# cvjena/mvlm

Hardware: NVIDIA B200
Metric: scans/sec (higher is better)
Workload: dtype bf16

## Files before the change

mvlm_b200/csrc/conv_epilogue.cuh:

```cuda
#pragma once
#include "conv_umma.cuh"

#include <type_traits>

#ifndef MVLM_FLOW_RES_BUDGET
#define MVLM_FLOW_RES_BUDGET 32
#endif

namespace mvlm {
namespace epi {

constexpr int kThreads = 352;
constexpr int kEpiWarps = 8;
constexpr int kTileW = 8;
constexpr int kMaxTileH = 32;
constexpr int kMTile = 128;
constexpr int kStageFloats = 16 * 36;
constexpr int kMaxCout = 256;
constexpr int kTraceTiles = 64;

enum : int { F_PRE = 1, F_RES1 = 2, F_RES2 = 4, F_RAW = 8, F_POST = 16, F_F32 = 32 , F_ARGMAX = 64,
              F_MID = 128 , F_POOL = 256 ,
              F_UP = 512 ,
              F_M64 = 1024 ,
              F_POST2 = 2048 ,
              F_POOLX = 4096 ,
              F_STAT = 8192  };
constexpr int F_HEAD = F_F32 | F_ARGMAX;

inline int feature_mask(const ConvEpilogue& e) {
  return (e.out_pre ? F_PRE : 0) | (e.res1 ? F_RES1 : 0) | (e.res2 ? F_RES2 : 0) | (e.out_raw ? F_RAW : 0) |
         (e.out_post ? F_POST : 0) | (e.out_f32 ? F_F32 : 0) | (e.argmax_keys ? F_ARGMAX : 0) |
         (e.mid_scale ? F_MID : 0) | (e.pool2 ? F_POOL : 0) | (e.res_up ? F_UP : 0) |
         (e.aux_mode == 1 ? F_POST2 : 0) | (e.aux_mode == 2 ? F_POOLX : 0);
}

#ifdef __CUDACC__

__device__ __forceinline__ uint32_t order_f32(float f) {
  const uint32_t b = __float_as_uint(f);
  return b ^ (static_cast<uint32_t>(static_cast<int32_t>(b) >> 31) | 0x80000000u);
}

__device__ __forceinline__ uint4 pack8(const float (&f)[8]) {
  __nv_bfloat162 a = __floats2bfloat162_rn(f[0], f[1]);
  __nv_bfloat162 b = __floats2bfloat162_rn(f[2], f[3]);
  __nv_bfloat162 c = __floats2bfloat162_rn(f[4], f[5]);
  __nv_bfloat162 d = __floats2bfloat162_rn(f[6], f[7]);
  uint4 r;
  r.x = *reinterpret_cast<uint32_t*>(&a);
// ... 81 lines not shown

struct EpiTrace {
  long long* trace = nullptr;
  int trace_i = 0;
  long long t0 = 0;
  bool on = false;
};
#define MVLM_EPI_TRACE(slot)                                                                              \
  do {                                                                                                    \
    if (tr.on && tr.trace && tr.trace_i < kTraceTiles) tr.trace[tr.trace_i * 16 + (slot)] = clock64() - tr.t0; \
  } while (0)

template <bool kFlow>
__device__ __forceinline__ uint4 load_res(const uint8_t* p) {
  if constexpr (kFlow) return __ldcg(reinterpret_cast<const uint4*>(p));
  else return *reinterpret_cast<const uint4*>(p);
}

template <int F, bool kFlow>
__device__ __forceinline__ void epilogue_tile(const ConvShape& s, const ConvEpilogue& e, const int tile_h,
                                              const ChannelParams& ep, const TileCoord& tc, const ImageSlots& is,
                                              uint64_t* t_full, const uint32_t parity, const uint32_t tmem_acc,
                                              float* stage, const int ew, const int lane_grp, const int lane,
                                              ArgmaxState& am, const bool prof, long long& w0, EpiTrace& tr) {
  constexpr bool WS = (F & F_M64) != 0;
  constexpr int kM = kMTile;
  constexpr int kChGrp = 32;
  constexpr int kPitch = 36;
  constexpr int kCols = 16;
  constexpr int kUnitRows = kCols / 8;
  static_assert(kCols * kPitch <= kStageFloats, "transpose buffer");
  const int rep_log2 = !WS ? 0 : (s.cout_pad <= 32 ? 2 : 1);
  const int n_cgrp = 4 >> rep_log2;
  const int cgrp = lane_grp & (n_cgrp - 1);
  const int replica = lane_grp >> (2 - rep_log2);
  const int n_units = max(1, tile_h / kUnitRows);
  const int upr = max(1, n_units >> rep_log2);
  const int upw = max(1, upr >> 1);
  const int u_local = (ew >> 2) * upw;
  const int u_begin = replica * upr + u_local;
  const int oh = s.h * e.up_sy, ow = s.w * e.up_sx;
  const int pj = lane >> 2;
  const int cq = (lane & 3) * 8;
  constexpr bool kBf16Out = (F & (F_PRE | F_RAW | F_POST)) != 0;
  const uint32_t rs_pre = static_cast<uint32_t>(s.w * e.pre_cs) * 2u, rs_res1 = static_cast<uint32_t>(s.w * e.res1_cs) * 2u;
  const uint32_t rs_res2 = static_cast<uint32_t>(s.w * e.res2_cs) * 2u;
  const uint32_t rs_up = static_cast<uint32_t>((s.w >> 1) * e.up_cs) * 2u;
// ... 187 lines not shown
        }
        if (r + 1 < upw) tmem_load(r + 1);
        if (y < s.h) {
          if (kBf16Out) {
            __syncwarp();
            if (r < 2) MVLM_EPI_TRACE(9 + 4 * r);
            uint4 pool_cur[2];
#pragma unroll
            for (int ip = 0; ip < 2; ++ip) {
              const int row = kUnitRows * r + ip;
              const bool valid = row < n_rows_ok;
              float f[8] = {0.f, 0.f, 0.f, 0.f, 0.f, 0.f, 0.f, 0.f};
              if (valid) {
                lds8(stage + (pj + 8 * ip) * kPitch + cq, f);
                if (F & F_PRE)
                  *reinterpret_cast<uint4*>(b_pre + static_cast<size_t>(row * rs_pre)) = affine_relu_pack8(f, pre_s, pre_t);
                if (F & F_RES1) add8(r1[r % kPref][ip], f);
                if (F & F_RES2) add8(r2[r % kPref][ip], f);
                if (F & F_UP) add8(ru[r % kPref][0], f);
              }
              if (F & (F_POOL | F_POOLX)) pool_cur[ip] = pack8(f);
              if (!(F & F_POOL) && valid) {
                if (F & F_RAW) *reinterpret_cast<uint4*>(b_raw + static_cast<size_t>(row * rs_raw)) = (F & F_POOLX) ? pool_cur[ip] : pack8(f);
                if (F & F_POST)
                  *reinterpret_cast<uint4*>(b_post + static_cast<size_t>(row * rs_post)) = affine_relu_pack8(f, post_s, post_t);
                if (F & F_POST2) {
                  float ax_s[8], ax_t[8], g[8] = {0.f, 0.f, 0.f, 0.f, 0.f, 0.f, 0.f, 0.f};
                  add8(pack8(f), g);
                  lds8(ep.mid_s + c0_ok, ax_s);
                  lds8(ep.mid_t + c0_ok, ax_t);
                  *reinterpret_cast<uint4*>(b_aux1 + static_cast<size_t>(row * rs_aux1)) = affine_relu_pack8(g, ax_s, ax_t);
                }
              }
            }
            if (r < 2) MVLM_EPI_TRACE(10 + 4 * r);
            if (F & (F_POOL | F_POOLX)) {
              {
                uint4 m = max_bf16x8(pool_cur[0], pool_cur[1]);
                uint4 o;
                o.x = __shfl_xor_sync(0xffffffffu, m.x, 4);
                o.y = __shfl_xor_sync(0xffffffffu, m.y, 4);
                o.z = __shfl_xor_sync(0xffffffffu, m.z, 4);
                o.w = __shfl_xor_sync(0xffffffffu, m.w, 4);
                m = max_bf16x8(m, o);
                const int prow = r;
                if (2 * prow < n_rows_ok && (pj & 1) == 0) {
                  if (F & F_POOL) {
                    if (F & F_RAW) *reinterpret_cast<uint4*>(b_raw + static_cast<size_t>(prow * rs_raw)) = m;
// ... 42 lines not shown
```

mvlm_b200/csrc/conv_umma.cu:

```cuda
#include "conv_epilogue.cuh"

#include <stdlib.h>

#include <algorithm>
#include <type_traits>
#include <atomic>

namespace mvlm {

namespace {

using namespace epi;
constexpr int kMaxHSlots = 4;
constexpr int kMaxWSlots = 12;
constexpr int kPoolBytes = 198 * 1024;

struct __align__(8) Barriers {
  uint64_t h_full[kMaxHSlots];
  uint64_t h_empty[kMaxHSlots];
  uint64_t w_full[kMaxWSlots];
  uint64_t w_empty[kMaxWSlots];
  uint64_t t_full[2];
  uint64_t t_empty[2];
  uint32_t tmem_base;
};
static_assert(sizeof(Barriers) <= 512, "barrier block");

struct EpiParams {
  float bias[kMaxCout];
  float mid_s[kMaxCout];
  float mid_t[kMaxCout];
  float pre_s[kMaxCout];
  float pre_t[kMaxCout];
  float post_s[kMaxCout];
  float post_t[kMaxCout];
};

constexpr int kSmemBytes = kPoolBytes + kEpiWarps * kStageFloats * 4 + 512 + static_cast<int>(sizeof(EpiParams)) +
                           1024 ;
static_assert(kSmemBytes <= 227 * 1024, "shared memory budget");

__device__ __forceinline__ TileCoord decode_tile(const ConvParams& p, int t) {
  TileCoord c;
  c.mt = t % p.n_nt;
  int r = t / p.n_nt;
  c.tx = r % p.tiles_x;
  r /= p.tiles_x;
  c.ty = r % p.tiles_y;
  c.img = r / p.tiles_y;
  return c;
}

struct TileIter {
  TileCoord c, d;
  int n_nt, tiles_x, tiles_y;
  __device__ __forceinline__ TileIter(const ConvParams& p, int t_begin, int t_step)
      : c(decode_tile(p, t_begin)), d(decode_tile(p, t_step)), n_nt(p.n_nt), tiles_x(p.tiles_x), tiles_y(p.tiles_y) {}
  __device__ __forceinline__ void next() {
// ... 2 lines not shown
    c.mt -= carry ? n_nt : 0;
    c.tx += d.tx + carry;
    carry = c.tx >= tiles_x ? 1 : 0;
    c.tx -= carry ? tiles_x : 0;
    c.ty += d.ty + carry;
    carry = c.ty >= tiles_y ? 1 : 0;
    c.ty -= carry ? tiles_y : 0;
    c.img += d.img + carry;
  }
};

template <int F>
__global__ void __launch_bounds__(kThreads, 1) conv_umma_kernel(const __grid_constant__ ConvParams p) {
  constexpr bool ARGMAX = (F & F_ARGMAX) != 0;
  extern __shared__ uint8_t smem_raw[];
  const uint32_t raw_addr = ptx::smem_u32(smem_raw);
  uint8_t* smem = smem_raw + ((1024u - (raw_addr & 1023u)) & 1023u);
  uint8_t* h_slots = smem;
  uint8_t* w_slots = smem + p.n_hslots * p.h_slot_bytes;
  float* stage_all = reinterpret_cast<float*>(smem + kPoolBytes);
  Barriers* bar = reinterpret_cast<Barriers*>(reinterpret_cast<uint8_t*>(stage_all) + kEpiWarps * kStageFloats * 4);
  EpiParams* ep = reinterpret_cast<EpiParams*>(reinterpret_cast<uint8_t*>(bar) + 512);

  const int warp = threadIdx.x >> 5;
  const int lane = threadIdx.x & 31;

  const ConvShape& s = p.s;
  const ConvEpilogue& e = p.e;
  const int n_chunks = (s.cin + 63) >> 6;
  const int n_hslots = p.n_hslots, n_wslots = p.n_wslots;
  const int halo_px = kTileW + s.kw - 1;
  const int halo_rows = p.tile_h + s.kh - 1;
  constexpr bool M64 = (F & F_M64) != 0;
  constexpr bool STAT = (F & F_STAT) != 0;
  constexpr int kM = M64 ? 64 : kMTile;
  const int w_rows = s.cout_pad < kM ? s.cout_pad : kM;
  const int mma_m = M64 ? (s.cout_pad <= 32 ? 32 : 64) : kMTile;
  const uint32_t w_tap_bytes = M64 ? 64u * 128u : ((static_cast<uint32_t>(w_rows) * 128u + 1023u) & ~1023u);
  const uint32_t w_slot_bytes = w_tap_bytes * static_cast<uint32_t>(M64 ? s.kh : 1);
  const bool w_stat = p.w_stationary != 0;

  int t_begin, t_end, t_step;
  if (ARGMAX) {
    const int per = (p.total_tiles + gridDim.x - 1) / gridDim.x;
    t_begin = blockIdx.x * per;
    t_end = min(p.total_tiles, t_begin + per);
    t_step = 1;
  } else {
    t_begin = blockIdx.x; t_end = p.total_tiles; t_step = gridDim.x;
  }

  for (int i = threadIdx.x; i < s.cout_pad; i += kThreads) {
    ep->bias[i] = e.bias ? e.bias[i] : 0.f;
    ep->mid_s[i] = e.mid_scale ? e.mid_scale[i] : (e.aux_scale ? e.aux_scale[i] : 1.f);
    ep->mid_t[i] = e.mid_scale ? e.mid_shift[i] : (e.aux_shift ? e.aux_shift[i] : 0.f);
    ep->pre_s[i] = e.out_pre ? e.pre_scale[i] : 0.f;
    ep->pre_t[i] = e.out_pre ? e.pre_shift[i] : 0.f;
    ep->post_s[i] = e.out_post ? e.post_scale[i] : 0.f;
    ep->post_t[i] = e.out_post ? e.post_shift[i] : 0.f;
  }
  if (warp == 0 && lane == 0) {
    ptx::tma_prefetch_desc(&p.tm_a);
    ptx::tma_prefetch_desc(&p.tm_b);
    if (p.tail) { ptx::tma_prefetch_desc(&p.tm_a2); ptx::tma_prefetch_desc(&p.tm_b2); }
    if (F & F_RES1) ptx::tma_prefetch_desc(&p.tm_r1);
    if (F & F_RES2) ptx::tma_prefetch_desc(&p.tm_r2);
    if (F & F_UP) ptx::tma_prefetch_desc(&p.tm_up);
    for (int i = 0; i < n_hslots; ++i) {
      ptx::mbar_init(&bar->h_full[i], 1);
      ptx::mbar_init(&bar->h_empty[i], 1);
    }
    for (int i = 0; i < n_wslots; ++i) {
      ptx::mbar_init(&bar->w_full[i], 1);
      ptx::mbar_init(&bar->w_empty[i], 1);
    }
    for (int i = 0; i < 2; ++i) {
      ptx::mbar_init(&bar->t_full[i], 1);
      ptx::mbar_init(&bar->t_empty[i], kEpiWarps);
    }
    ptx::fence_mbar_init();
  }
  if (warp == 1) {
    ptx::tmem_alloc(&bar->tmem_base, 512);
    ptx::tmem_relinquish();
  }
  ptx::tc_fence_before();
  __syncthreads();
  ptx::tc_fence_after();
  asm volatile("griddepcontrol.wait;" ::: "memory");
  asm volatile("griddepcontrol.launch_dependents;" ::: "memory");
// ... 18 lines not shown
        const int x0 = tc.tx * kTileW + s.x_off0;
        const int y0 = tc.ty * p.tile_h + s.y_off0;
        for (int c = 0; c < n_chunks; ++c) {
          const bool is_tail = p.tail != 0 && c == n_chunks - 1;
          const uint32_t row_b = is_tail ? static_cast<uint32_t>(p.tail) * 2u : 128u;
          timed_wait(&bar->h_empty[sh], ph ^ 1, prof, w0);
          ptx::mbar_expect_tx(&bar->h_full[sh], static_cast<uint32_t>(halo_rows * halo_px) * row_b);
          ptx::tma_load_4d(is_tail ? &p.tm_a2 : &p.tm_a, &bar->h_full[sh], h_slots + sh * p.h_slot_bytes, c * 64, x0, y0, tc.img);
          if (c == 0) MVLM_TRACE(0);
          if (++sh == n_hslots) { sh = 0; ph ^= 1; }
        }
        if constexpr ((F & (F_RES1 | F_RES2 | F_UP)) != 0) {
          const int xa = tc.tx * kTileW, ya = tc.ty * p.tile_h, c_lo = tc.mt * kM;
          if (F & F_RES1) ptx::tma_prefetch_l2_4d(&p.tm_r1, c_lo, xa, ya, tc.img);
          if (F & F_RES2) ptx::tma_prefetch_l2_4d(&p.tm_r2, c_lo, xa, ya, tc.img);
          if (F & F_UP) ptx::tma_prefetch_l2_4d(&p.tm_up, c_lo, xa >> 1, ya >> 1, tc.img);
        }
        ++trace_i;
      }
      if (prof) { p.prof[blockIdx.x * 8 + 0] = w0; p.prof[blockIdx.x * 8 + 7] = clock64() - t_kernel0; }
    }
  } else if (warp == 10) {
    if (ptx::elect_one() && (p.debug_mode & 1) == 0) {
      int sw = 0;
      uint32_t pw = 0;
      for (int t = t_begin; t < t_end; t += t_step) {
        const int mt = t % p.n_nt;
        for (int c = 0; c < n_chunks; ++c) {
          const bool is_tail = p.tail != 0 && c == n_chunks - 1;
          const void* tmb = is_tail ? &p.tm_b2 : &p.tm_b;
          const uint32_t row_b = is_tail ? static_cast<uint32_t>(p.tail) * 2u : 128u;
          const uint32_t wb = static_cast<uint32_t>(w_rows) * row_b;
          if constexpr (M64) {
            for (int kx = 0; kx < s.kw; ++kx) {
              if (!w_stat) timed_wait(&bar->w_empty[sw], pw ^ 1, prof, w1);
              ptx::mbar_expect_tx(&bar->w_full[sw], wb * static_cast<uint32_t>(s.kh));
              for (int ky = 0; ky < s.kh; ++ky)
                ptx::tma_load_2d(tmb, &bar->w_full[sw], w_slots + sw * w_slot_bytes + ky * w_tap_bytes,
                                 (kx * s.kh + ky) * s.cin + c * 64, mt * kM);
              if (++sw == n_wslots) { sw = 0; pw ^= 1; }
            }
          } else
          for (int tap = 0; tap < s.kw * s.kh; ++tap) {
            if (!w_stat) timed_wait(&bar->w_empty[sw], pw ^ 1, prof, w1);
            ptx::mbar_expect_tx(&bar->w_full[sw], wb);
            ptx::tma_load_2d(tmb, &bar->w_full[sw], w_slots + sw * w_slot_bytes, tap * s.cin + c * 64, mt * kM);
// ... 6 lines not shown
      }
      if (prof) p.prof[blockIdx.x * 8 + 1] = w1;
    }
  } else if (warp == 1) {
    if (ptx::elect_one()) {
      const uint32_t idesc = ptx::umma_idesc_bf16(mma_m, p.tile_h * kTileW);
      const bool live = (p.debug_mode & 1) == 0;
      const int n_kx = s.kw, n_ky = s.kh;
      const uint32_t tail_row_b = p.tail ? static_cast<uint32_t>(p.tail) * 2u : 128u;
      const uint32_t tail_swz = !p.tail ? 2u : (p.tail == 16 ? 6u : 4u);
      const uint64_t a_hi_full = static_cast<uint64_t>(((8u * 128u) >> 4) | (1u << 14) | (2u << 29)) << 32;
      const uint64_t b_hi_full = static_cast<uint64_t>(((static_cast<uint32_t>(halo_px) * 128u) >> 4) | (1u << 14) | (2u << 29)) << 32;
      const uint64_t a_hi_tail = static_cast<uint64_t>(((8u * tail_row_b) >> 4) | (1u << 14) | (tail_swz << 29)) << 32;
      const uint64_t b_hi_tail = static_cast<uint64_t>(((static_cast<uint32_t>(halo_px) * tail_row_b) >> 4) | (1u << 14) | (tail_swz << 29)) << 32;
      const uint32_t h_lo0 = (ptx::smem_u32(h_slots) >> 4) | (1u << 16), h_step = static_cast<uint32_t>(p.h_slot_bytes) >> 4;
      const uint32_t w_lo0 = (ptx::smem_u32(w_slots) >> 4) | (1u << 16), w_step = w_slot_bytes >> 4;
      const int last_chunk = n_chunks - 1;
      const int nk_last = (s.cin - last_chunk * 64) >= 64 ? 4 : ((s.cin - last_chunk * 64) >> 4);
      int sh = 0, sw = 0;
      uint32_t ph = 0, pw = 0;
      int acc = 0;
      uint32_t pacc = 0;
      bool w_wait = live;
      for (int t = t_begin; t < t_end; t += t_step) {
        timed_wait(&bar->t_empty[acc], pacc ^ 1, prof, w1);
        ptx::tc_fence_after();
        MVLM_TRACE(2);
        const uint32_t d = tmem_base + static_cast<uint32_t>(acc * 256);
        uint32_t accumulate = 0;
        for (int c = 0; c < n_chunks; ++c) {
          const bool is_tail = p.tail != 0 && c == last_chunk;
          const int nk = c == last_chunk ? nk_last : 4;
          const uint32_t rb16 = (is_tail ? tail_row_b : 128u) >> 4;
          const uint64_t a_hi = is_tail ? a_hi_tail : a_hi_full;
          const uint64_t b_hi = is_tail ? b_hi_tail : b_hi_full;
          const uint32_t ky_step = static_cast<uint32_t>(halo_px) * rb16;
          if (live) timed_wait(&bar->h_full[sh], ph, prof, w0);
          if (c == 0) MVLM_TRACE(3);
          uint32_t x_col = h_lo0 + static_cast<uint32_t>(sh) * h_step;
          if (STAT && !w_wait && (nk == 4 || nk == 2 || nk == 1)) {
            auto taps = [&](auto nk_c, auto kk_c) __attribute__((always_inline)) {
              constexpr int NK = decltype(nk_c)::value;
              constexpr int KK = decltype(kk_c)::value;
              constexpr uint32_t kRb16 = NK * 2;
              const uint32_t tap16 = M64 ? (64u * 128u >> 4) : w_step;
              const uint32_t w_base = w_lo0 + static_cast<uint32_t>(c * KK * KK) * tap16;
#pragma unroll
              for (int tap = 0; tap < KK * KK; ++tap) {
                const uint32_t x_lo = x_col + static_cast<uint32_t>(((tap % KK) * (kTileW + KK - 1) + tap / KK)) * kRb16;
                const uint32_t w_lo = w_base + static_cast<uint32_t>(tap) * tap16;
#pragma unroll
// ... 39 lines not shown
            uint32_t x_lo = x_col;
            for (int ky = 0; ky < n_ky; ++ky, x_lo += ky_step) {
              if (w_wait) timed_wait(&bar->w_full[sw], w_stat ? 0u : pw, prof, w0);
              const uint32_t w_lo = w_lo0 + static_cast<uint32_t>(sw) * w_step;
              auto mma = [&](int k, uint32_t en) __attribute__((always_inline)) {
                if constexpr (M64) ptx::umma_ws_bf16(d, a_hi | (w_lo + 2 * k), b_hi | (x_lo + 2 * k), idesc, en);
                else ptx::umma_bf16(d, a_hi | (w_lo + 2 * k), b_hi | (x_lo + 2 * k), idesc, en);
              };
              mma(0, accumulate);
              if (nk == 4) {
                mma(1, 1u); mma(2, 1u); mma(3, 1u);
              } else {
                for (int k = 1; k < nk; ++k) mma(k, 1u);
              }
              accumulate = 1;
              if (live && !w_stat) ptx::umma_commit(&bar->w_empty[sw]);
              if (++sw == n_wslots) { sw = 0; pw ^= 1; }
            }
          }
          if (live) ptx::umma_commit(&bar->h_empty[sh]);
          if (++sh == n_hslots) { sh = 0; ph ^= 1; }
        }
        ptx::umma_commit(&bar->t_full[acc]);
        MVLM_TRACE(4);
        ++trace_i;
        if (w_stat) w_wait = false;
        if (++acc == 2) { acc = 0; pacc ^= 1; }
      }
      if (prof) { p.prof[blockIdx.x * 8 + 2] = w0; p.prof[blockIdx.x * 8 + 3] = w1; p.prof[blockIdx.x * 8 + 4] = clock64() - t_kernel0; }
    }
  } else {
    float* stage = stage_all + (warp - 2) * kStageFloats;
    const ChannelParams cp = {ep->bias, ep->mid_s, ep->mid_t, ep->pre_s, ep->pre_t, ep->post_s, ep->post_t};
    int acc = 0;
    uint32_t pacc = 0;
    ArgmaxState am;
    EpiTrace tr;
    tr.trace = trace; tr.t0 = t_kernel0; tr.on = warp == 2 && lane == 0;
    TileIter it(p, t_begin, t_step);
    for (int t = t_begin; t < t_end; t += t_step, it.next()) {
      const TileCoord tc = it.c;
      const ImageSlots is = {tc.img, tc.img, tc.img, tc.img, tc.img, tc.img, tc.img, tc.img};
      tr.trace_i = trace_i;
      if (p.debug_mode & 2) {
        timed_wait(&bar->t_full[acc], pacc, prof, w0);
        ptx::tc_fence_after();
      } else {
        epilogue_tile<F, false>(s, e, p.tile_h, cp, tc, is, &bar->t_full[acc], pacc,
                                tmem_base + static_cast<uint32_t>(acc * 256), stage, warp - 2, warp & 3, lane, am, prof, w0,
                                tr);
      }
      ptx::tc_fence_before();
      __syncwarp();
      if (lane == 0) ptx::mbar_arrive(&bar->t_empty[acc]);
      if (warp == 2 && lane == 0) MVLM_TRACE(6);
      ++trace_i;
      if (++acc == 2) { acc = 0; pacc ^= 1; }
    }
    epilogue_argmax_flush<F>(s, e, warp & 3, lane, am);
    if (prof && warp == 2 && lane == 0) { p.prof[blockIdx.x * 8 + 5] = w0; p.prof[blockIdx.x * 8 + 6] = clock64() - t_kernel0; }
  }

#undef MVLM_TRACE
  ptx::tc_fence_before();
  __syncthreads();
  if (warp == 1) {
    ptx::tc_fence_after();
    ptx::tmem_dealloc(tmem_base, 512);
  }
}

typedef CUresult (*EncodeTiledFn)(CUtensorMap*, CUtensorMapDataType, cuuint32_t, void*,
                                  const cuuint64_t*, const cuuint64_t*, const cuuint32_t*,
                                  const cuuint32_t*, CUtensorMapInterleave, CUtensorMapSwizzle,
                                  CUtensorMapL2promotion, CUtensorMapFloatOOBfill);

EncodeTiledFn get_encode_fn() {
// ... 164 lines not shown
      cuuint32_t estr[4] = {1, 1, 1, 1};
      return enc(tm, CU_TENSOR_MAP_DATA_TYPE_BFLOAT16, 4, const_cast<__nv_bfloat16*>(base + co), gdim, gstr, box, estr,
                 CU_TENSOR_MAP_INTERLEAVE_NONE, CU_TENSOR_MAP_SWIZZLE_NONE, CU_TENSOR_MAP_L2_PROMOTION_L2_128B,
                 CU_TENSOR_MAP_FLOAT_OOB_FILL_NONE) == CUDA_SUCCESS;
    };
    const bool ok = res_map(&p.tm_r1, e.res1, e.res1_co, e.res1_cs, s.h, s.w, kTileW, tile_h) &&
                    res_map(&p.tm_r2, e.res2, e.res2_co, e.res2_cs, s.h, s.w, kTileW, tile_h) &&
                    res_map(&p.tm_up, e.res_up, e.up_co, e.up_cs, s.h >> 1, s.w >> 1, kTileW / 2, std::max(1, tile_h / 2));
    if (!ok) {
      set_error("conv_plan: cuTensorMapEncodeTiled(residual) failed (cout_pad=%d w=%d h=%d)", s.cout_pad, s.w, s.h);
      return MVLM_E_CUDA;
    }
  }
  p.tiles_x = ceil_div(s.w, kTileW);
  p.tiles_y = ceil_div(s.h, tile_h);
  p.n_nt = s.cout_pad <= 64 ? 1 : ceil_div(s.cout_pad, kMTile);
  p.total_tiles = s.n * p.tiles_x * p.tiles_y * p.n_nt;
  p.prof = nullptr;
  p.debug_mode = 0;
  *out = p;
  return MVLM_OK;
}

void conv_set_profile_buffer(long long* dev_buf) { g_prof_buf = dev_buf; }
void conv_set_debug_mode(int mode) { g_debug_mode = mode; }

int conv_launch(const ConvParams& p_in, cudaStream_t stream) {
  ConvParams p = p_in;
  p.prof = g_prof_buf;
  p.debug_mode = g_debug_mode;
  const ConvEpilogue& e = p.e;
  const int f = feature_mask(e);
  const bool m64 = p.s.cout_pad <= 64;
  const bool stat = m64 && p.w_stationary && p.s.kw == 3 && p.s.kh == 3;
#define MVLM_CASE_BOTH(FLAGS) \
  case (FLAGS):               \
    return m64 ? (stat ? launch_t<(FLAGS) | F_M64 | F_STAT>(p, stream) : launch_t<(FLAGS) | F_M64>(p, stream)) : launch_t<(FLAGS)>(p, stream)
#define MVLM_CASE_128(FLAGS) \
  case (FLAGS):              \
    if (!m64) return launch_t<(FLAGS)>(p, stream); \
    break
  if (f == F_ARGMAX && !m64 && p.w_stationary && p.s.kw == 2 && p.s.kh == 2) return launch_t<F_ARGMAX | F_STAT>(p, stream);
  switch (f) {
    MVLM_CASE_BOTH(F_PRE | F_RES1 | F_RAW | F_POST);
    MVLM_CASE_BOTH(F_PRE | F_RES1 | F_RAW);
    MVLM_CASE_BOTH(F_RES1 | F_RAW | F_POST);
    MVLM_CASE_BOTH(F_RES1 | F_RAW);
    MVLM_CASE_BOTH(F_RAW);
    MVLM_CASE_128(F_PRE);
    MVLM_CASE_128(F_RES1 | F_RES2 | F_RAW | F_POST);
    MVLM_CASE_128(F_ARGMAX);
    MVLM_CASE_BOTH(F_F32);
    MVLM_CASE_BOTH(F_F32 | F_ARGMAX);
    MVLM_CASE_BOTH(F_MID | F_PRE | F_POST);
    MVLM_CASE_BOTH(F_POOL | F_PRE | F_RES1 | F_RAW | F_POST);
    MVLM_CASE_BOTH(F_POOL | F_RES1 | F_RAW | F_POST);
    MVLM_CASE_BOTH(F_POOL | F_RAW);
    MVLM_CASE_128(F_PRE | F_RES1 | F_RES2 | F_RAW | F_POST);
    MVLM_CASE_BOTH(F_UP | F_PRE | F_RES1 | F_RAW | F_POST);
    MVLM_CASE_BOTH(F_UP | F_PRE | F_RES1 | F_RAW);
    MVLM_CASE_BOTH(F_UP | F_RES1 | F_RAW | F_POST);
    MVLM_CASE_BOTH(F_UP | F_RES1 | F_RAW);
    MVLM_CASE_BOTH(F_POST2 | F_PRE | F_RES1 | F_RAW | F_POST);
    MVLM_CASE_BOTH(F_POST2 | F_RES1 | F_RAW | F_POST);
// ... 12 lines not shown
```

mvlm_b200/csrc/conv_umma.cuh:

```cuda
#pragma once
#include "common.cuh"

namespace mvlm {

struct ConvEpilogue {
  const float* bias = nullptr;
  const float* mid_scale = nullptr;
  const float* mid_shift = nullptr;
  const float* pre_scale = nullptr;
  const float* pre_shift = nullptr;
  __nv_bfloat16* out_pre = nullptr;
  int pre_cs = 0, pre_co = 0;
  const __nv_bfloat16* res1 = nullptr;
  int res1_cs = 0, res1_co = 0;
  const __nv_bfloat16* res2 = nullptr;
  int res2_cs = 0, res2_co = 0;
  const __nv_bfloat16* res_up = nullptr;
  int up_cs = 0, up_co = 0;
  __nv_bfloat16* out_raw = nullptr;
  int raw_cs = 0, raw_co = 0;
  const float* post_scale = nullptr;
  const float* post_shift = nullptr;
  __nv_bfloat16* out_post = nullptr;
  int post_cs = 0, post_co = 0;
// ... 18 lines not shown
  int in_cs = 0;
  const __nv_bfloat16* wpacked = nullptr;
  int cout_pad = 0;
  int n_tile = 0;
  int kh = 3, kw = 3;
  int y_off0 = -1, x_off0 = -1;
};

struct alignas(64) ConvParams {
  CUtensorMap tm_a;
  CUtensorMap tm_b;
  CUtensorMap tm_a2;
  CUtensorMap tm_b2;
  CUtensorMap tm_r1, tm_r2, tm_up;
  int tail;
  ConvShape s;
  ConvEpilogue e;
  int tiles_x, tiles_y, n_nt, total_tiles;
  int tile_h;
  int h_slot_bytes, n_hslots, n_wslots;
  int w_stationary;
  long long* prof;
  int debug_mode;
};

int conv_plan(const ConvShape& s, const ConvEpilogue& e, ConvParams* out);
int conv_launch(const ConvParams& p, cudaStream_t stream);
constexpr int kConvTraceTiles = 64;
constexpr int kConvProfInts = 148 * 8 + kConvTraceTiles * 16;
void conv_set_profile_buffer(long long* dev_buf);
void conv_set_debug_mode(int mode);

}
```

mvlm_b200/csrc/hourglass.cu:

```cuda
#include "hourglass.cuh"

#include <math.h>
#include <stdlib.h>

#include <algorithm>

namespace mvlm {

namespace {

__global__ void fold_bn_kernel(const float* w, const float* b, const float* m, const float* v, float eps, int n,
                               float* scale, float* shift) {
  const int i = blockIdx.x * blockDim.x + threadIdx.x;
  if (i >= n) return;
  const float s = w[i] / sqrtf(v[i] + eps);
  scale[i] = s;
  shift[i] = b[i] - m[i] * s;
}

__global__ void pack_weight_kernel(const float* __restrict__ w, int cout, int cin, int k, int cout_pad, int cin_pad,
                                   __nv_bfloat16* __restrict__ out) {
  const long long total = 1ll * cout_pad * k * k * cin_pad;
  for (long long i = blockIdx.x * 1ll * blockDim.x + threadIdx.x; i < total; i += 1ll * gridDim.x * blockDim.x) {
    const int ci = static_cast<int>(i % cin_pad);
// ... 149 lines not shown
        ++j;
      }
    }
    size_t best = free_list.size();
    for (size_t j = 0; j < free_list.size(); ++j)
      if (free_list[j].bytes >= b.bytes && (best == free_list.size() || free_list[j].bytes < free_list[best].bytes)) best = j;
    if (best < free_list.size()) {
      b.offset = free_list[best].off;
      free_list[best].off += b.bytes;
      free_list[best].bytes -= b.bytes;
      if (free_list[best].bytes == 0) free_list.erase(free_list.begin() + best);
    } else {
      b.offset = top;
      top += b.bytes;
    }
    ws_needed_ = std::max(ws_needed_, b.offset + b.bytes);
    ws_needed_ = std::max(ws_needed_, top);
    live.push_back(id);
  }
}

static int op_out_rows(const NetOp& op) {
  switch (op.kind) {
    case NetOp::CONV: return op.is_head ? -1 : op.h;
    case NetOp::POOL: return op.h / 2;
    case NetOp::BNRELU: return op.h;
    default: return -1;
  }
}

void HourglassNet::push_op(const NetOp& op) {
  const int rows = op_out_rows(op);
  const bool in_window = flow_on_ && rows >= flow_lo_ && rows <= flow_hi_;
  if (!in_window) {
    cur_seg_ = -1;
  } else if (cur_seg_ < 0 || cur_seg_layers_ >= kFlowMaxLayers) {
    cur_seg_ = n_segs_++;
    cur_seg_layers_ = 0;
  }
  if (in_window) ++cur_seg_layers_;
  ops_.push_back(op);
  op_seg_.push_back(cur_seg_);
}

HourglassNet::T HourglassNet::alloc(int h, int w, int c) {
  T t;
  t.h = h; t.w = w; t.c = c;
// ... 95 lines not shown
    packed(wname + ".weight", cout, cin_real, k, cout_pad, cin, &dw);
    if (with_bias) bias(wname + ".bias", cout, cout_pad, &db);
  }
  if (!dry_) {
    ConvShape s;
    s.in = in.p; s.n = V_; s.h = in.h; s.w = in.w; s.cin = cin; s.in_cs = in.c;
    const __nv_bfloat16* wp;
    int rc = packed(wname + ".weight", cout, cin_real, k, cout_pad, cin, &wp);
    if (rc) return rc;
    s.wpacked = wp; s.cout_pad = cout_pad; s.n_tile = n_tile; s.kh = k; s.kw = k;
    s.y_off0 = -(k / 2); s.x_off0 = -(k / 2);
    if (with_bias) {
      rc = bias(wname + ".bias", cout, cout_pad, &e.bias);
      if (rc) return rc;
    }
    rc = conv_plan(s, e, &op.conv);
    if (rc) return rc;
  }
  push_op(op);
  return MVLM_OK;
}

int HourglassNet::rb(const std::string& p, T x, T a_in, T ar, int cin, int cout, const char* post_bn, T* post_act,
                     T* y_out, T* pool_raw, const T* up_low, const RbAux* aux) {
  const int h = a_in.h, w = a_in.w;
  T y = alloc(h, w, cout);
  T skip = x;
  int rc;
  if (cin != cout) {
    ConvEpilogue e;
    e.out_raw = y.p; e.raw_cs = cout; e.raw_co = 0;
    rc = emit_conv("rb.resample", ar, cin, p + ".resample.2", cout, cout, cout < 128 ? cout : 128, 1, e, false);
    if (rc) return rc;
    skip = y;
  }
  const float *ps = nullptr, *pt = nullptr;
  if (post_bn) {
    rc = bn(post_bn, cout, &ps, &pt);
    if (rc) return rc;
    *post_act = pool_raw ? alloc(h / 2, w / 2, cout) : alloc(h, w, cout);
  }
  if (pool_raw) *pool_raw = alloc(h / 2, w / 2, cout);
  const float *as = nullptr, *at = nullptr;
  if (aux) {
    rc = bn(aux->bn, cout, &as, &at);
    if (rc) return rc;
    *aux->out1 = aux->mode == 2 ? alloc(h / 2, w / 2, cout) : alloc(h, w, cout);
    if (aux->mode == 2) *aux->out2 = alloc(h / 2, w / 2, cout);
  }
  const int c1 = cout / 2, c2 = cout / 4;
  T a1 = alloc(h, w, c1);
  T a2 = alloc(h, w, c2);
// ... 158 lines not shown
  cudaStreamDestroy(build_stream_);
  build_stream_ = nullptr;
  if (rc) return rc;
  MVLM_CHECK_CUDA(ce);
  return MVLM_OK;
}

void HourglassNet::probe(const char* name, const T& t) {
  probes[name] = {t.p, t.h, t.w, t.c};
  if (layout_pass_ && keep_probes_ && t.p) {
    const size_t off = static_cast<size_t>(reinterpret_cast<const uint8_t*>(t.p) - kFakeBase);
    for (Buf& b : bufs_)
      if (b.fake_off == off) b.pinned = true;
  }
}

int HourglassNet::emit() {
  const int h = H_, w = W_, cin = cin_;
  ops_.clear(); flops_ = 0.0; probes.clear();
  op_seg_.clear(); segs_.clear(); seg_info_.clear(); cur_seg_ = -1; n_segs_ = 0; cur_seg_layers_ = 0;
  int rc;
  const int F = 256, h2 = h / 2, w2 = w / 2;

  T a_c2 = alloc(h, w, 64), ar_c2 = alloc(h, w, 64);
  T img16 = alloc(h, w, 16);
  {
    note_use(img16.p);
    NetOp op;
    op.kind = NetOp::STEM;
    op.out_raw = img16.p; op.h = h; op.w = w; op.c = cin;
    push_op(op);
    flops_ += 2.0 * 64 * cin * 9 * h * w;
    note_use(img16.p); note_use(a_c2.p); note_use(ar_c2.p);
    NetOp cv;
    cv.kind = NetOp::CONV;
    cv.tag = "conv1";
    cv.h = h; cv.w = w;
    if (layout_pass_) {
      param_alloc(sizeof(__nv_bfloat16) * 64 * 9 * 16);
      const float* dummy;
      bias("conv1.bias", 64, 64, &dummy);
      bn("bn1", 64, &dummy, &dummy);
      bn("conv2.bn1", 64, &dummy, &dummy);
      bn("conv2.resample.0", 64, &dummy, &dummy);
    }
    if (!dry_) {
      const float* w1 = nullptr;
      if ((rc = sd_get("conv1.weight", 64ll * cin * 9, &w1))) return rc;
      __nv_bfloat16* wp = static_cast<__nv_bfloat16*>(param_alloc(sizeof(__nv_bfloat16) * 64 * 9 * 16));
      MVLM_REQUIRE(wp, "hourglass: parameter arena exhausted (conv1)");
      pack_stem_weight_kernel<<<36, 256, 0, build_stream_>>>(w1, 64, cin, 64, wp);
      MVLM_CHECK_CUDA(cudaGetLastError());
      ConvShape s;
      s.in = img16.p; s.n = V_; s.h = h; s.w = w; s.cin = 16; s.in_cs = 16;
      s.wpacked = wp; s.cout_pad = 64; s.n_tile = 64; s.kh = 3; s.kw = 3; s.y_off0 = -1; s.x_off0 = -1;
      ConvEpilogue e;
      if ((rc = bias("conv1.bias", 64, 64, &e.bias))) return rc;
      if ((rc = bn("bn1", 64, &e.mid_scale, &e.mid_shift))) return rc;
      if ((rc = bn("conv2.bn1", 64, &e.pre_scale, &e.pre_shift))) return rc;
      if ((rc = bn("conv2.resample.0", 64, &e.post_scale, &e.post_shift))) return rc;
      e.out_pre = a_c2.p; e.pre_cs = 64; e.pre_co = 0;
      e.out_post = ar_c2.p; e.post_cs = 64; e.post_co = 0;
      if ((rc = conv_plan(s, e, &cv.conv))) return rc;
    }
    push_op(cv);
  }
  T none, y2, y3, r3, a3, a4, a_h1, ar4;
  T x1;
  if ((rc = rb("conv2", none, a_c2, ar_c2, 64, 128, "conv3.bn1", &a3, &y2, &x1))) return rc;
  probe("x1", x1);
  if (fuse_elt_) {
    RbAux aux = {1, "conv4.resample.0", &ar4, nullptr};
    if ((rc = rb("conv3", x1, a3, none, 128, 128, "conv4.bn1", &a4, &y3, nullptr, nullptr, &aux))) return rc;
    probe("y3", y3);
  } else {
    if ((rc = rb("conv3", x1, a3, none, 128, 128, "conv4.bn1", &a4, &y3))) return rc;
    probe("y3", y3);
    ar4 = alloc(h2, w2, 128);
    note_use(y3.p); note_use(ar4.p);
    NetOp op;
    op.kind = NetOp::BNRELU;
    op.in0 = y3.p; op.out_act = ar4.p; op.h = h2; op.w = w2; op.c = 128;
    if ((rc = bn("conv4.resample.0", 128, &op.scale, &op.shift))) return rc;
    push_op(op);
  }
  T p1, pa1, p2, pa2;
  RbAux aux4 = {2, "hg1.rb2.bn1", &p1, &pa1};
  if ((rc = rb("conv4", y3, a4, ar4, 128, F, "hg1.rb1.bn1", &a_h1, &r3, nullptr, nullptr, fuse_elt_ ? &aux4 : nullptr))) return rc;
  probe("r3", r3);
  T hg1;
  if ((rc = hourglass("hg1", r3, a_h1, &hg1, fuse_elt_ ? &p1 : nullptr, fuse_elt_ ? &pa1 : nullptr))) return rc;
  probe("hg1", hg1);
// ... 384 lines not shown
```

mvlm_b200/csrc/hourglass.cuh:

```cuda
#pragma once
#include <map>
#include <set>
#include <string>
#include <vector>

#include "conv_flow.cuh"
#include "conv_umma.cuh"
#include "stages.cuh"

namespace mvlm {

struct SdEntry {
  const float* p = nullptr;
  long long numel = -1;
};
typedef std::map<std::string, SdEntry> StateDict;

struct NetOp {
  enum Kind { CONV, POOL, BNRELU, STEM, MEMSET, PEAKS } kind;
  ConvParams conv;
  const __nv_bfloat16* in0 = nullptr;
  const __nv_bfloat16* in1 = nullptr;
  __nv_bfloat16* out_raw = nullptr;
  __nv_bfloat16* out_act = nullptr;
  const float* scale = nullptr;
  const float* shift = nullptr;
  int h = 0, w = 0, c = 0;
  void* ptr = nullptr;
  size_t bytes = 0;
  bool is_head = false;
  const char* tag = "";
};

class HourglassNet {
 public:
  HourglassNet() = default;
  ~HourglassNet();
  int build(const StateDict* sd, int n_landmarks, int cin, int n_views, int h, int w,
            void* workspace, size_t workspace_bytes, bool dry);
  int forward(const unsigned char* img_u8, const float* img_f32, float* out_heatmaps, float* out_peaks,
              cudaStream_t stream);
  int run_op(NetOp& op, const unsigned char* img_u8, const float* img_f32, float* out_heatmaps, float* out_peaks,
             cudaStream_t stream);
  int run_step(size_t i, const unsigned char* img_u8, const float* img_f32, float* out_heatmaps, float* out_peaks,
               cudaStream_t stream);
  int forward_graph(const unsigned char* img_u8, const float* img_f32, float* out_heatmaps, float* out_peaks,
                    cudaStream_t stream);

  int set_selection_method(int method);
  int forward_keys(const unsigned char* img_u8, const float* img_f32, unsigned long long* out_keys, cudaStream_t stream);

  int profile_ops(const unsigned char* img_u8, const float* img_f32, float* out_peaks, int reps, float* ms_out,
                  double* roles_out, int trace_op, long long* trace_out, cudaStream_t stream);
// ... 21 lines not shown
    bool pinned = false;
  };
  int emit();
  void note_use(const void* p);
  void note_conv(const void* in, const ConvEpilogue& e);
  void assign_offsets();
  void probe(const char* name, const T& t);
  void* param_alloc(size_t bytes);
  unsigned char* params_ = nullptr;
  size_t param_off_ = 0, param_cap_ = 0;
  std::set<std::string> bn_seen_;
  cudaStream_t build_stream_ = nullptr;
  static constexpr size_t kMaxGraphs = 8;
  std::vector<Buf> bufs_;
  size_t fake_off_ = 0, ws_needed_ = 0, next_buf_ = 0;
  bool layout_pass_ = false, keep_probes_ = false, reuse_ = true, fuse_elt_ = false;
  int bn(const std::string& name, int c, const float** scale, const float** shift);
  int packed(const std::string& name, int cout, int cin, int k, int cout_pad, int cin_pad, const __nv_bfloat16** out);
  int bias(const std::string& name, int cout, int cout_pad, const float** out);
  int emit_conv(const char* tag, T in, int cin, const std::string& wname, int cout, int cout_pad, int n_tile, int k,
                ConvEpilogue e, bool with_bias);
  struct RbAux { int mode; const char* bn; T* out1; T* out2; };
  int rb(const std::string& p, T x, T a_in, T ar, int cin, int cout, const char* post_bn, T* post_act, T* y_out,
         T* pool_raw = nullptr, const T* up_low = nullptr, const RbAux* aux = nullptr);
  int hourglass(const std::string& p, T x, T a_x, T* out, const T* in_pooled = nullptr, const T* in_pooled_act = nullptr);
  int emit_pool(T in, T out_raw, const char* bn_name, T out_act);

  void push_op(const NetOp& op);
  int build_segments();
  bool flow_on_ = false;
  int flow_lo_ = 1, flow_hi_ = 32;
  int cur_seg_layers_ = 0;
  int flow_tiles_ = 64;
  int flow_interleave_ = 3;
  int cur_seg_ = -1, n_segs_ = 0;
  std::vector<int> op_seg_;
  std::vector<FlowSegment> segs_;
  struct SegInfo { int batch = 1, n_layers = 0, first_op = -1; };
  std::vector<SegInfo> seg_info_;
  float* zeros_ = nullptr;
  float* ones_ = nullptr;

  const StateDict* sd_ = nullptr;
  int sd_get(const std::string& name, long long numel, const float** out) const;
  bool dry_ = true;
  int V_ = 0, H_ = 0, W_ = 0, L_ = 0, Lp_ = 0, cin_ = 0;
  uint8_t* ws_ = nullptr;
// ... 17 lines not shown
```

Before: 64.23.

## Chain conv1 with the conv2 1x1 resample GEMM inside one UMMA kernel

Fuses the stem's 3x3 conv1 with the following 1x1 resample conv. The post-activated tile is staged in swizzled shared memory, a second UMMA against preloaded W2 writes into a separate TMEM region, and a second epilogue pass stores the 128-channel result. This drops the separate resample launch and the global round trip of the activated intermediate. In exchange it adds more barriers, halves the accumulator column stride, and leaves less shared memory for the operand rings.

```diff
diff --git a/mvlm_b200/csrc/conv_epilogue.cuh b/mvlm_b200/csrc/conv_epilogue.cuh
--- a/mvlm_b200/csrc/conv_epilogue.cuh
+++ b/mvlm_b200/csrc/conv_epilogue.cuh
@@ -25,7 +25,8 @@
               F_M64 = 1024 ,
               F_POST2 = 2048 ,
               F_POOLX = 4096 ,
-              F_STAT = 8192  };
+              F_STAT = 8192 ,
+              F_CHAIN = 16384  };
 constexpr int F_HEAD = F_F32 | F_ARGMAX;
 
 inline int feature_mask(const ConvEpilogue& e) {
@@ -153,7 +154,8 @@
                                               const ChannelParams& ep, const TileCoord& tc, const ImageSlots& is,
                                               uint64_t* t_full, const uint32_t parity, const uint32_t tmem_acc,
                                               float* stage, const int ew, const int lane_grp, const int lane,
-                                              ArgmaxState& am, const bool prof, long long& w0, EpiTrace& tr) {
+                                              ArgmaxState& am, const bool prof, long long& w0, EpiTrace& tr,
+                                              uint8_t* stg = nullptr) {
   constexpr bool WS = (F & F_M64) != 0;
   constexpr int kM = kMTile;
   constexpr int kChGrp = 32;
@@ -387,8 +389,12 @@
               if (F & (F_POOL | F_POOLX)) pool_cur[ip] = pack8(f);
               if (!(F & F_POOL) && valid) {
                 if (F & F_RAW) *reinterpret_cast<uint4*>(b_raw + static_cast<size_t>(row * rs_raw)) = (F & F_POOLX) ? pool_cur[ip] : pack8(f);
-                if (F & F_POST)
+                if constexpr ((F & F_CHAIN) != 0) {
+                  const int n = (kUnitRows * u_begin + row) * kTileW + pj;
+                  *reinterpret_cast<uint4*>(stg + n * 128 + (((c0 >> 3) ^ pj) << 4)) = affine_relu_pack8(f, post_s, post_t);
+                } else if (F & F_POST) {
                   *reinterpret_cast<uint4*>(b_post + static_cast<size_t>(row * rs_post)) = affine_relu_pack8(f, post_s, post_t);
+                }
                 if (F & F_POST2) {
                   float ax_s[8], ax_t[8], g[8] = {0.f, 0.f, 0.f, 0.f, 0.f, 0.f, 0.f, 0.f};
                   add8(pack8(f), g);
diff --git a/mvlm_b200/csrc/conv_umma.cu b/mvlm_b200/csrc/conv_umma.cu
--- a/mvlm_b200/csrc/conv_umma.cu
+++ b/mvlm_b200/csrc/conv_umma.cu
@@ -14,6 +14,9 @@
 constexpr int kMaxHSlots = 4;
 constexpr int kMaxWSlots = 12;
 constexpr int kPoolBytes = 198 * 1024;
+constexpr int kChainWBytes = kMTile * 128;
+constexpr int kChainStageBytes = kMaxTileH * kTileW * 128;
+constexpr int kChainBytes = kChainWBytes + 2 * kChainStageBytes;
 
 struct __align__(8) Barriers {
   uint64_t h_full[kMaxHSlots];
@@ -22,6 +25,9 @@
   uint64_t w_empty[kMaxWSlots];
   uint64_t t_full[2];
   uint64_t t_empty[2];
+  uint64_t s_full[2], s_empty[2];
+  uint64_t r_full, r_empty;
+  uint64_t w2_full;
   uint32_t tmem_base;
 };
 static_assert(sizeof(Barriers) <= 512, "barrier block");
@@ -34,6 +40,7 @@
   float pre_t[kMaxCout];
   float post_s[kMaxCout];
   float post_t[kMaxCout];
+  float zero[kMTile];
 };
 
 constexpr int kSmemBytes = kPoolBytes + kEpiWarps * kStageFloats * 4 + 512 + static_cast<int>(sizeof(EpiParams)) +
@@ -82,6 +89,11 @@
   Barriers* bar = reinterpret_cast<Barriers*>(reinterpret_cast<uint8_t*>(stage_all) + kEpiWarps * kStageFloats * 4);
   EpiParams* ep = reinterpret_cast<EpiParams*>(reinterpret_cast<uint8_t*>(bar) + 512);
 
+  constexpr bool CHAIN = (F & F_CHAIN) != 0;
+  uint8_t* const c_w2 = smem + kPoolBytes - kChainBytes;
+  uint8_t* const c_stg = c_w2 + kChainWBytes;
+  constexpr uint32_t kAccCols = CHAIN ? 128u : 256u;
+
   const int warp = threadIdx.x >> 5;
   const int lane = threadIdx.x & 31;
 
@@ -116,9 +128,11 @@
     ep->mid_t[i] = e.mid_scale ? e.mid_shift[i] : (e.aux_shift ? e.aux_shift[i] : 0.f);
     ep->pre_s[i] = e.out_pre ? e.pre_scale[i] : 0.f;
     ep->pre_t[i] = e.out_pre ? e.pre_shift[i] : 0.f;
-    ep->post_s[i] = e.out_post ? e.post_scale[i] : 0.f;
-    ep->post_t[i] = e.out_post ? e.post_shift[i] : 0.f;
-  }
+    ep->post_s[i] = (e.out_post || CHAIN) ? e.post_scale[i] : 0.f;
+    ep->post_t[i] = (e.out_post || CHAIN) ? e.post_shift[i] : 0.f;
+  }
+  if (CHAIN)
+    for (int i = threadIdx.x; i < kMTile; i += kThreads) ep->zero[i] = 0.f;
   if (warp == 0 && lane == 0) {
     ptx::tma_prefetch_desc(&p.tm_a);
     ptx::tma_prefetch_desc(&p.tm_b);
@@ -126,6 +140,16 @@
     if (F & F_RES1) ptx::tma_prefetch_desc(&p.tm_r1);
     if (F & F_RES2) ptx::tma_prefetch_desc(&p.tm_r2);
     if (F & F_UP) ptx::tma_prefetch_desc(&p.tm_up);
+    if (CHAIN) {
+      ptx::tma_prefetch_desc(&p.tm_w2);
+      for (int i = 0; i < 2; ++i) {
+        ptx::mbar_init(&bar->s_full[i], kEpiWarps);
+        ptx::mbar_init(&bar->s_empty[i], 1);
+      }
+      ptx::mbar_init(&bar->r_full, 1);
+      ptx::mbar_init(&bar->r_empty, kEpiWarps);
+      ptx::mbar_init(&bar->w2_full, 1);
+    }
     for (int i = 0; i < n_hslots; ++i) {
       ptx::mbar_init(&bar->h_full[i], 1);
       ptx::mbar_init(&bar->h_empty[i], 1);
@@ -190,6 +214,10 @@
     }
   } else if (warp == 10) {
     if (ptx::elect_one() && (p.debug_mode & 1) == 0) {
+      if (CHAIN) {
+        ptx::mbar_expect_tx(&bar->w2_full, kChainWBytes);
+        ptx::tma_load_2d(&p.tm_w2, &bar->w2_full, c_w2, 0, 0);
+      }
       int sw = 0;
       uint32_t pw = 0;
       for (int t = t_begin; t < t_end; t += t_step) {
@@ -242,11 +270,28 @@
       int acc = 0;
       uint32_t pacc = 0;
       bool w_wait = live;
-      for (int t = t_begin; t < t_end; t += t_step) {
+      const uint32_t idesc2 = ptx::umma_idesc_bf16(kMTile, p.tile_h * kTileW);
+      const uint32_t w2_lo = (ptx::smem_u32(c_w2) >> 4) | (1u << 16);
+      const uint32_t stg_lo0 = (ptx::smem_u32(c_stg) >> 4) | (1u << 16);
+      auto chain_gemm = [&](int j) __attribute__((always_inline)) {
+        const int sb = j & 1;
+        timed_wait(&bar->s_full[sb], static_cast<uint32_t>(j >> 1) & 1u, prof, w0);
+        timed_wait(&bar->r_empty, static_cast<uint32_t>(j & 1) ^ 1u, prof, w1);
+        if (j == 0 && live) timed_wait(&bar->w2_full, 0u, prof, w0);
+        ptx::tc_fence_after();
+        const uint32_t b_lo = stg_lo0 + static_cast<uint32_t>(sb) * (kChainStageBytes >> 4);
+#pragma unroll
+        for (int k = 0; k < 4; ++k)
+          ptx::umma_bf16(tmem_base + 256u, a_hi_full | (w2_lo + 2 * k), a_hi_full | (b_lo + 2 * k), idesc2, k > 0 ? 1u : 0u);
+        ptx::umma_commit(&bar->s_empty[sb]);
+        ptx::umma_commit(&bar->r_full);
+      };
+      int j_tile = 0;
+      for (int t = t_begin; t < t_end; t += t_step, ++j_tile) {
         timed_wait(&bar->t_empty[acc], pacc ^ 1, prof, w1);
         ptx::tc_fence_after();
         MVLM_TRACE(2);
-        const uint32_t d = tmem_base + static_cast<uint32_t>(acc * 256);
+        const uint32_t d = tmem_base + static_cast<uint32_t>(acc) * kAccCols;
         uint32_t accumulate = 0;
         for (int c = 0; c < n_chunks; ++c) {
           const bool is_tail = p.tail != 0 && c == last_chunk;
@@ -332,11 +377,13 @@
           if (++sh == n_hslots) { sh = 0; ph ^= 1; }
         }
         ptx::umma_commit(&bar->t_full[acc]);
+        if (CHAIN && j_tile > 0) chain_gemm(j_tile - 1);
         MVLM_TRACE(4);
         ++trace_i;
         if (w_stat) w_wait = false;
         if (++acc == 2) { acc = 0; pacc ^= 1; }
       }
+      if (CHAIN && j_tile > 0) chain_gemm(j_tile - 1);
       if (prof) { p.prof[blockIdx.x * 8 + 2] = w0; p.prof[blockIdx.x * 8 + 3] = w1; p.prof[blockIdx.x * 8 + 4] = clock64() - t_kernel0; }
     }
   } else {
@@ -347,22 +394,42 @@
     ArgmaxState am;
     EpiTrace tr;
     tr.trace = trace; tr.t0 = t_kernel0; tr.on = warp == 2 && lane == 0;
+    ConvShape s2 = s;
+    s2.cout_pad = kMTile;
+    ConvEpilogue e2;
+    e2.out_raw = p.out2; e2.raw_cs = kMTile;
+    const ChannelParams cp2 = {ep->zero, ep->zero, ep->zero, ep->zero, ep->zero, ep->zero, ep->zero};
+    EpiTrace tr2;
     TileIter it(p, t_begin, t_step);
-    for (int t = t_begin; t < t_end; t += t_step, it.next()) {
+    int j_tile = 0;
+    for (int t = t_begin; t < t_end; t += t_step, it.next(), ++j_tile) {
       const TileCoord tc = it.c;
       const ImageSlots is = {tc.img, tc.img, tc.img, tc.img, tc.img, tc.img, tc.img, tc.img};
+      const int sb = j_tile & 1;
       tr.trace_i = trace_i;
+      if (CHAIN) timed_wait(&bar->s_empty[sb], (static_cast<uint32_t>(j_tile >> 1) & 1u) ^ 1u, prof, w0);
       if (p.debug_mode & 2) {
         timed_wait(&bar->t_full[acc], pacc, prof, w0);
         ptx::tc_fence_after();
       } else {
         epilogue_tile<F, false>(s, e, p.tile_h, cp, tc, is, &bar->t_full[acc], pacc,
-                                tmem_base + static_cast<uint32_t>(acc * 256), stage, warp - 2, warp & 3, lane, am, prof, w0,
-                                tr);
+                                tmem_base + static_cast<uint32_t>(acc) * kAccCols, stage, warp - 2, warp & 3, lane, am, prof,
+                                w0, tr, c_stg + sb * kChainStageBytes);
       }
       ptx::tc_fence_before();
+      if (CHAIN) ptx::fence_proxy_async();
       __syncwarp();
-      if (lane == 0) ptx::mbar_arrive(&bar->t_empty[acc]);
+      if (lane == 0) {
+        ptx::mbar_arrive(&bar->t_empty[acc]);
+        if (CHAIN) ptx::mbar_arrive(&bar->s_full[sb]);
+      }
+      if (CHAIN) {
+        epilogue_tile<F_RAW, false>(s2, e2, p.tile_h, cp2, tc, is, &bar->r_full, static_cast<uint32_t>(j_tile & 1),
+                                    tmem_base + 256u, stage, warp - 2, warp & 3, lane, am, prof, w0, tr2);
+        ptx::tc_fence_before();
+        __syncwarp();
+        if (lane == 0) ptx::mbar_arrive(&bar->r_empty);
+      }
       if (warp == 2 && lane == 0) MVLM_TRACE(6);
       ++trace_i;
       if (++acc == 2) { acc = 0; pacc ^= 1; }
@@ -573,6 +640,38 @@
   return MVLM_OK;
 }
 
+int conv_plan_chain(const ConvShape& s, const ConvEpilogue& e, const __nv_bfloat16* w2, __nv_bfloat16* out2,
+                    ConvParams* out) {
+  MVLM_REQUIRE(w2 && out2 && (reinterpret_cast<uintptr_t>(w2) & 15) == 0, "conv_plan_chain: null or misaligned w2 / out2");
+  MVLM_REQUIRE(s.cout_pad == 64 && s.cin <= 64 && s.kh == 3 && s.kw == 3 && !e.out_post && e.post_scale && e.post_shift &&
+                   feature_mask(e) == (F_MID | F_PRE),
+               "conv_plan_chain: needs a 3x3 conv with cin <= 64, cout_pad 64 and a bias -> mid -> {pre, post} epilogue");
+  ConvParams p;
+  int rc = conv_plan(s, e, &p);
+  if (rc) return rc;
+  MVLM_REQUIRE(p.w_stationary, "conv_plan_chain: weights must be stationary");
+  const int row_b = p.tail ? p.tail * 2 : 128;
+  p.h_slot_bytes = ((kTileW + s.kw - 1) * (p.tile_h + s.kh - 1) * row_b + 1023) & ~1023;
+  const int w_ring = p.n_wslots * 64 * 128 * s.kh;
+  const int room = kPoolBytes - kChainBytes - w_ring;
+  p.n_hslots = std::min(kMaxHSlots, room / p.h_slot_bytes);
+  MVLM_REQUIRE(p.n_hslots >= 2, "conv_plan_chain: operand rings do not fit");
+  EncodeTiledFn enc = get_encode_fn();
+  cuuint64_t gdim[2] = {64, (cuuint64_t)kMTile};
+  cuuint64_t gstr[1] = {64 * 2};
+  cuuint32_t box[2] = {64, (cuuint32_t)kMTile};
+  cuuint32_t estr[2] = {1, 1};
+  if (enc(&p.tm_w2, CU_TENSOR_MAP_DATA_TYPE_BFLOAT16, 2, const_cast<__nv_bfloat16*>(w2), gdim, gstr, box, estr,
+          CU_TENSOR_MAP_INTERLEAVE_NONE, CU_TENSOR_MAP_SWIZZLE_128B, CU_TENSOR_MAP_L2_PROMOTION_L2_256B,
+          CU_TENSOR_MAP_FLOAT_OOB_FILL_NONE) != CUDA_SUCCESS) {
+    set_error("conv_plan_chain: cuTensorMapEncodeTiled(W2) failed");
+    return MVLM_E_CUDA;
+  }
+  p.out2 = out2;
+  *out = p;
+  return MVLM_OK;
+}
+
 void conv_set_profile_buffer(long long* dev_buf) { g_prof_buf = dev_buf; }
 void conv_set_debug_mode(int mode) { g_debug_mode = mode; }
 
@@ -591,6 +690,7 @@
   case (FLAGS):              \
     if (!m64) return launch_t<(FLAGS)>(p, stream); \
     break
+  if (p.out2) return launch_t<F_MID | F_PRE | F_POST | F_M64 | F_STAT | F_CHAIN>(p, stream);
   if (f == F_ARGMAX && !m64 && p.w_stationary && p.s.kw == 2 && p.s.kh == 2) return launch_t<F_ARGMAX | F_STAT>(p, stream);
   switch (f) {
     MVLM_CASE_BOTH(F_PRE | F_RES1 | F_RAW | F_POST);
diff --git a/mvlm_b200/csrc/conv_umma.cuh b/mvlm_b200/csrc/conv_umma.cuh
--- a/mvlm_b200/csrc/conv_umma.cuh
+++ b/mvlm_b200/csrc/conv_umma.cuh
@@ -64,9 +64,13 @@
   int w_stationary;
   long long* prof;
   int debug_mode;
+  CUtensorMap tm_w2;
+  __nv_bfloat16* out2;
 };
 
 int conv_plan(const ConvShape& s, const ConvEpilogue& e, ConvParams* out);
+int conv_plan_chain(const ConvShape& s, const ConvEpilogue& e, const __nv_bfloat16* w2, __nv_bfloat16* out2,
+                    ConvParams* out);
 int conv_launch(const ConvParams& p, cudaStream_t stream);
 constexpr int kConvTraceTiles = 64;
 constexpr int kConvProfInts = 148 * 8 + kConvTraceTiles * 16;
diff --git a/mvlm_b200/csrc/hourglass.cu b/mvlm_b200/csrc/hourglass.cu
--- a/mvlm_b200/csrc/hourglass.cu
+++ b/mvlm_b200/csrc/hourglass.cu
@@ -195,7 +195,7 @@
 
 static int op_out_rows(const NetOp& op) {
   switch (op.kind) {
-    case NetOp::CONV: return op.is_head ? -1 : op.h;
+    case NetOp::CONV: return (op.is_head || op.chained) ? -1 : op.h;
     case NetOp::POOL: return op.h / 2;
     case NetOp::BNRELU: return op.h;
     default: return -1;
@@ -337,12 +337,12 @@
 }
 
 int HourglassNet::rb(const std::string& p, T x, T a_in, T ar, int cin, int cout, const char* post_bn, T* post_act,
-                     T* y_out, T* pool_raw, const T* up_low, const RbAux* aux) {
+                     T* y_out, T* pool_raw, const T* up_low, const RbAux* aux, const T* resampled) {
   const int h = a_in.h, w = a_in.w;
-  T y = alloc(h, w, cout);
-  T skip = x;
+  T y = resampled ? *resampled : alloc(h, w, cout);
+  T skip = resampled ? y : x;
   int rc;
-  if (cin != cout) {
+  if (cin != cout && !resampled) {
     ConvEpilogue e;
     e.out_raw = y.p; e.raw_cs = cout; e.raw_co = 0;
     rc = emit_conv("rb.resample", ar, cin, p + ".resample.2", cout, cout, cout < 128 ? cout : 128, 1, e, false);
@@ -547,7 +547,7 @@
   int rc;
   const int F = 256, h2 = h / 2, w2 = w / 2;
 
-  T a_c2 = alloc(h, w, 64), ar_c2 = alloc(h, w, 64);
+  T a_c2 = alloc(h, w, 64), y_c2 = alloc(h, w, 128);
   T img16 = alloc(h, w, 16);
   {
     note_use(img16.p);
@@ -555,19 +555,22 @@
     op.kind = NetOp::STEM;
     op.out_raw = img16.p; op.h = h; op.w = w; op.c = cin;
     push_op(op);
-    flops_ += 2.0 * 64 * cin * 9 * h * w;
-    note_use(img16.p); note_use(a_c2.p); note_use(ar_c2.p);
+    flops_ += 2.0 * 64 * cin * 9 * h * w + 2.0 * 128 * 64 * h * w;
+    note_use(img16.p); note_use(a_c2.p); note_use(y_c2.p);
     NetOp cv;
     cv.kind = NetOp::CONV;
-    cv.tag = "conv1";
+    cv.tag = "conv1+resample";
+    cv.chained = true;
     cv.h = h; cv.w = w;
     if (layout_pass_) {
       param_alloc(sizeof(__nv_bfloat16) * 64 * 9 * 16);
       const float* dummy;
+      const __nv_bfloat16* dummy_w;
       bias("conv1.bias", 64, 64, &dummy);
       bn("bn1", 64, &dummy, &dummy);
       bn("conv2.bn1", 64, &dummy, &dummy);
       bn("conv2.resample.0", 64, &dummy, &dummy);
+      packed("conv2.resample.2.weight", 128, 64, 1, 128, 64, &dummy_w);
     }
     if (!dry_) {
       const float* w1 = nullptr;
@@ -585,14 +588,18 @@
       if ((rc = bn("conv2.bn1", 64, &e.pre_scale, &e.pre_shift))) return rc;
       if ((rc = bn("conv2.resample.0", 64, &e.post_scale, &e.post_shift))) return rc;
       e.out_pre = a_c2.p; e.pre_cs = 64; e.pre_co = 0;
-      e.out_post = ar_c2.p; e.post_cs = 64; e.post_co = 0;
-      if ((rc = conv_plan(s, e, &cv.conv))) return rc;
+      const __nv_bfloat16* w2 = nullptr;
+      if ((rc = packed("conv2.resample.2.weight", 128, 64, 1, 128, 64, &w2))) return rc;
+      if ((rc = conv_plan_chain(s, e, w2, y_c2.p, &cv.conv))) return rc;
     }
     push_op(cv);
   }
+  probe("img16", img16);
+  probe("a_c2", a_c2);
+  probe("y_c2", y_c2);
   T none, y2, y3, r3, a3, a4, a_h1, ar4;
   T x1;
-  if ((rc = rb("conv2", none, a_c2, ar_c2, 64, 128, "conv3.bn1", &a3, &y2, &x1))) return rc;
+  if ((rc = rb("conv2", none, a_c2, none, 64, 128, "conv3.bn1", &a3, &y2, &x1, nullptr, nullptr, &y_c2))) return rc;
   probe("x1", x1);
   if (fuse_elt_) {
     RbAux aux = {1, "conv4.resample.0", &ar4, nullptr};
diff --git a/mvlm_b200/csrc/hourglass.cuh b/mvlm_b200/csrc/hourglass.cuh
--- a/mvlm_b200/csrc/hourglass.cuh
+++ b/mvlm_b200/csrc/hourglass.cuh
@@ -29,6 +29,7 @@
   void* ptr = nullptr;
   size_t bytes = 0;
   bool is_head = false;
+  bool chained = false;
   const char* tag = "";
 };
 
@@ -96,7 +97,7 @@
                 ConvEpilogue e, bool with_bias);
   struct RbAux { int mode; const char* bn; T* out1; T* out2; };
   int rb(const std::string& p, T x, T a_in, T ar, int cin, int cout, const char* post_bn, T* post_act, T* y_out,
-         T* pool_raw = nullptr, const T* up_low = nullptr, const RbAux* aux = nullptr);
+         T* pool_raw = nullptr, const T* up_low = nullptr, const RbAux* aux = nullptr, const T* resampled = nullptr);
   int hourglass(const std::string& p, T x, T a_x, T* out, const T* in_pooled = nullptr, const T* in_pooled_act = nullptr);
   int emit_pool(T in, T out_raw, const char* bn_name, T out_act);
 
```

Result: no change. 64.34 (median of 6 runs) (+0.2%).
